# ofsoundof/NTIRE2022_ESR

Measured on AMD Instinct MI355X. Metric: images/sec (256x256->1024x1024 x4), higher is better.
Workload: dtype f32

## Files before the change

ntire2022_esr_amd/csrc/esr_wino.hip:

```cpp
#include <hip/hip_runtime.h>
#include <stddef.h>
#include <math.h>
#include <stdint.h>
#include <string.h>
#include <type_traits>

#include "esr_hip.h"
#include "esr_internal.h"

typedef float f32x4 __attribute__((ext_vector_type(4)));
typedef float f32x2 __attribute__((ext_vector_type(2)));
typedef int wn_i32x4 __attribute__((ext_vector_type(4)));

namespace {

constexpr int WN_THREADS = 256;
constexpr int WN_TILE = 16;
constexpr int WN_HALO = WN_TILE + 2;
constexpr int WN_PAIR = 37;
constexpr int WN_PLANE = 9 * WN_PAIR;
constexpr int WN_RAW_SLOTS = 2 * WN_PLANE;
constexpr int WN_LAST_LANES = WN_RAW_SLOTS - 640;
constexpr int WN_RAW_BYTES = WN_RAW_SLOTS * 16;
constexpr int WN_U_BYTES = 16 * 1024;
constexpr int WN_RING = 3;
constexpr int WN_RAW_OFF = WN_RING * WN_U_BYTES;
constexpr int WN_BIAS_OFF = WN_RAW_OFF + WN_RING * WN_RAW_BYTES;
constexpr int WN_LDS = WN_BIAS_OFF + 256;
static_assert(2 * WN_LDS <= 160 * 1024, "two blocks per CU");
constexpr int WN_MAX_BLOCKS = 512;
constexpr unsigned WN_OOB = 0x80000000u;
constexpr int WN_BARRIER_POS = 12;
constexpr int WN_FIRST_SHARE = 9;

struct WinoK {
    const float* x;
    const float* up;
    const float* bias;
    const float* res;
    float* y0;
    float* y1;
    int N, H, W;
    int nchunks, nhalves;
    unsigned up_bytes;
    int in_pitch, in_coff;
    int res_pitch, res_coff;
    int y0_pitch, y0_coff, y1_pitch, y1_coff;
    int cout_store, split;
    int act;
    float slope;
    int res_mode;
    int tiles_x, tiles_y;
    unsigned magic_x, magic_y;
    int y1_blk;
    int first_share;
    unsigned pix_floats;
    unsigned in_base;
    unsigned chunk_stride;
};

__device__ __forceinline__ unsigned wn_div(unsigned n, unsigned d, unsigned magic) { return d == 1 ? n : __umulhi(n, magic); }

__device__ __forceinline__ wn_i32x4 wn_rsrc(const void* base, size_t bytes)
{
    wn_i32x4 r;
    r.x = __builtin_amdgcn_readfirstlane((int)(size_t)base);
    r.y = __builtin_amdgcn_readfirstlane((int)(((size_t)base >> 32) & 0xffff));
    r.z = __builtin_amdgcn_readfirstlane((int)bytes);
    r.w = 0x00020000;
    return r;
}

template <int OFF>
__device__ __forceinline__ void wn_dma16(unsigned m0_base, unsigned voff, wn_i32x4 rsrc, unsigned soff)
{
    asm volatile("s_nop 0\n\tbuffer_load_dwordx4 %0, %1, %2 offen offset:%3 lds"
                 :: "v"(voff), "s"(rsrc), "s"(soff), "n"(OFF), "{m0}"(m0_base) : "memory");
}

__device__ __forceinline__ float wn_act1(float v, int act, float slope)
{
    switch (act) {
        case ESR_ACT_LRELU: return fmaxf(v, slope * v);
        case ESR_ACT_RELU: return fmaxf(v, 0.f);
        case ESR_ACT_GELU: return 0.5f * v * (1.f + erff(v * 0.70710678118654752440f));
        default: return v;
    }
}

template <int ACT>
__device__ __forceinline__ f32x4 wn_act4(f32x4 v, int act, float slope)
{
    if (ACT == ESR_ACT_LRELU) {
        const f32x4 m = v * slope;
        v.x = fmaxf(v.x, m.x); v.y = fmaxf(v.y, m.y); v.z = fmaxf(v.z, m.z); v.w = fmaxf(v.w, m.w);
    } else if (ACT < 0) {
        v.x = wn_act1(v.x, act, slope); v.y = wn_act1(v.y, act, slope);
        v.z = wn_act1(v.z, act, slope); v.w = wn_act1(v.w, act, slope);
    }
    return v;
}

__device__ __forceinline__ int wn_slot(int ly, int lx) { return (ly >> 1) * WN_PAIR + (ly & 1) * WN_HALO + lx; }

__device__ __forceinline__ f32x2 wn_lds_b64(unsigned addr)
{
    typedef const volatile __attribute__((address_space(3))) f32x2* lds_ptr;
    return *(lds_ptr)addr;
}

__device__ __forceinline__ f32x2 wn_sub2(f32x2 a, f32x2 b)
{
    f32x2 r;
    asm("v_pk_add_f32 %0, %1, %2 neg_lo:[0,1] neg_hi:[0,1]" : "=v"(r) : "v"(a), "v"(b));
    return r;
}

__device__ __forceinline__ void wn_pair_planes(f32x4& v0, f32x4& v1)
{
#pragma unroll
    for (int e = 0; e < 4; ++e) {
        const float a = v0[e], b = v1[e];
        const auto r = __builtin_amdgcn_permlane32_swap(__builtin_bit_cast(unsigned, a), __builtin_bit_cast(unsigned, b), false, false);
        const unsigned r0 = r[0], r1 = r[1];
        v0[e] = __builtin_bit_cast(float, r0);
        v1[e] = __builtin_bit_cast(float, r1);
    }
}

__device__ __forceinline__ f32x2 wn_add2(f32x2 a, f32x2 b)
{
    f32x2 r;
    asm("v_pk_add_f32 %0, %1, %2" : "=v"(r) : "v"(a), "v"(b));
    return r;
}

__device__ __forceinline__ void wn_mfma(f32x4& acc, float a, float b)
{
    asm("v_mfma_f32_16x16x4_f32 %0, %1, %2, %0" : "+v"(acc) : "v"(a), "v"(b));
}
__device__ __forceinline__ void wn_mfma_drain(f32x4& acc) { asm volatile("s_nop 15\n\ts_nop 3" : "+v"(acc)); }

#define WN_PIN(x) asm volatile("" : "+v"(x))

template <int ACT, int RES, int OUT>
__global__ __launch_bounds__(WN_THREADS, 2) void wino_f32_kernel(const WinoK p)
{
    __shared__ __attribute__((aligned(16))) char smem[WN_LDS];

    const int tid = threadIdx.x;
    const int lane = tid & 63;
    const int wv = __builtin_amdgcn_readfirstlane(tid >> 6);
    const int j = lane & 15, g = lane >> 4;
    const int tx = j & 7, ty = j >> 3;
    const unsigned smem_lds = (unsigned)(size_t)(__attribute__((address_space(3))) char*)smem;

    const int nwork = p.N * p.tiles_y * p.tiles_x * p.nhalves;
    const int G = gridDim.x;
    const bool classes = p.first_share != 8 && (G & 15) == 0;
    const int GC = classes ? G >> 1 : G;
    const bool second = classes && (int)blockIdx.x >= GC;
    const int n_first = classes ? (int)(((long)nwork * p.first_share / 16) & ~1L) : nwork;
    const int cbase = second ? n_first : 0, cend = second || !classes ? nwork : n_first;
    const int bl = second ? (int)blockIdx.x - GC : (int)blockIdx.x;
    auto work_index = [&](int k) -> int {
        const int base = cbase + k * GC;
        if (base >= cend) return -1;
        int off = bl;
        if ((GC & 7) == 0 && base + GC <= cend) off = (bl & 7) * (GC >> 3) + (bl >> 3);
        const int t = base + off;
        return t < cend ? t : -1;
    };

    struct Ctx { int n, x0, y0, half; unsigned voff[3]; };
    auto setup = [&](int work, Ctx& c) {
        if (work < 0) {
            c.n = 0; c.x0 = 0; c.y0 = 0; c.half = 0;
            c.voff[0] = c.voff[1] = c.voff[2] = WN_OOB;
            return;
        }
        const unsigned t = p.nhalves == 2 ? (unsigned)work >> 1 : (unsigned)work;
        c.half = p.nhalves == 2 ? work & 1 : 0;
        const unsigned tq = wn_div(t, (unsigned)p.tiles_x, p.magic_x);
        const unsigned txi = t - tq * p.tiles_x;
        c.n = (int)wn_div(tq, (unsigned)p.tiles_y, p.magic_y);
        const unsigned tyi = tq - (unsigned)c.n * p.tiles_y;
        c.x0 = (int)txi * WN_TILE;
        c.y0 = (int)tyi * WN_TILE;
#pragma unroll
        for (int i = 0; i < 3; ++i) {
            const int item = (wv * 3 + (wv == 3 && i == 2 ? 0 : i)) * 64 + lane;
            const int half = item >= WN_PLANE ? 1 : 0;
            const int slot = item - half * WN_PLANE;
            const int pr = slot / WN_PAIR, rem = slot - pr * WN_PAIR;
            const int odd = rem >= WN_HALO ? 1 : 0;
            const int ly = 2 * pr + odd, lx = rem - odd * WN_HALO;
            const int gy = c.y0 - 1 + ly, gx = c.x0 - 1 + lx;
            const bool ok = item < WN_RAW_SLOTS && rem < 2 * WN_HALO && gy >= 0 && gy < p.H && gx >= 0 && gx < p.W;
            c.voff[i] = (ok ? ((unsigned)(gy * p.W + gx) * p.pix_floats + 4u * half) * 4u + p.in_base : WN_OOB) - (i == 1 ? 1024u : 0u);
        }
    };
    const size_t img_bytes = (size_t)p.H * p.W * p.in_pitch * 4;
    const wn_i32x4 ursrc = wn_rsrc(p.up, p.up_bytes);
    const bool live1 = wv != 3 || lane < WN_LAST_LANES;
    const unsigned raw_m0 = smem_lds + (unsigned)(WN_RAW_OFF + wv * 3 * 1024);
    const unsigned raw_m0_2 = raw_m0 + (wv == 3 ? 0u : 2048u);
    const unsigned u_m0 = smem_lds + (unsigned)(wv * 4 * 1024);

    auto issue_raw = [&](int i, int rs, wn_i32x4 xr, int chunk, unsigned v) __attribute__((always_inline)) {
        const unsigned soff = (unsigned)chunk * p.chunk_stride;
        const unsigned ro = (unsigned)(rs * WN_RAW_BYTES);
        if (i == 0) wn_dma16<0>(raw_m0 + ro, v, xr, soff);
        else if (i == 1) { if (live1) wn_dma16<1024>(raw_m0 + ro, v, xr, soff); }
        else wn_dma16<0>(raw_m0_2 + ro, v, xr, soff);
    };
    auto image_rsrc = [&](int n) { return wn_rsrc(p.x + (size_t)n * (img_bytes / 4), img_bytes); };
    auto issue_u = [&](int i, int us, int half, int chunk, bool live) __attribute__((always_inline)) {
        const unsigned soff = (unsigned)((chunk * p.nhalves + half) * WN_U_BYTES + wv * 4 * 1024);
        const unsigned vo = live ? (unsigned)lane * 16u : WN_OOB;
        const unsigned m = u_m0 + (unsigned)(us * WN_U_BYTES);
        if (i == 0) wn_dma16<0>(m, vo, ursrc, soff);
        else if (i == 1) wn_dma16<1024>(m, vo, ursrc, soff);
        else if (i == 2) wn_dma16<2048>(m, vo, ursrc, soff);
        else wn_dma16<3072>(m, vo, ursrc, soff);
    };

    const int raw_lane = (g >> 1) * (WN_PLANE * 16) + wn_slot(4 * wv + 2 * ty, 2 * tx) * 16 + (g & 1) * 8;
    const int u_lane = lane * 16;

    auto raw_row = [&](unsigned rb, int r, f32x2 (&d)[4]) __attribute__((always_inline)) {
#pragma unroll
        for (int dx = 0; dx < 4; ++dx)
            d[dx] = wn_lds_b64(rb + ((r >> 1) * WN_PAIR + (r & 1) * WN_HALO + dx) * 16);
    };
    auto row_pass = [&](f32x2 (&V)[16], int r, const f32x2 (&d)[4]) __attribute__((always_inline)) {
        V[4 * r + 0] = wn_sub2(d[0], d[2]);
        V[4 * r + 1] = wn_add2(d[1], d[2]);
        V[4 * r + 2] = wn_sub2(d[2], d[1]);
        V[4 * r + 3] = wn_sub2(d[1], d[3]);
    };
    auto col_pass = [&](f32x2 (&V)[16], int c) __attribute__((always_inline)) {
        const f32x2 w0 = V[c], w1 = V[4 + c], w2 = V[8 + c], w3 = V[12 + c];
        V[c] = wn_sub2(w0, w2);
        V[4 + c] = wn_add2(w1, w2);
        V[8 + c] = wn_sub2(w2, w1);
        V[12 + c] = wn_sub2(w1, w3);
    };

    int k = 0;
    int work = work_index(0);
    if (work < 0) return;
    Ctx cur, nxt;
    setup(work, cur);
    int wn = work_index(1);
    setup(wn, nxt);

    {
        const wn_i32x4 xr = image_rsrc(cur.n);
#pragma unroll
        for (int c = 0; c < 3; ++c)
#pragma unroll
            for (int i = 0; i < 3; ++i) issue_raw(i, c, xr, c, cur.voff[i]);
#pragma unroll
        for (int i = 0; i < 4; ++i) issue_u(i, 0, cur.half, 0, true);
    }
    if (tid < p.nhalves * 8) *reinterpret_cast<f32x4*>(smem + WN_BIAS_OFF + tid * 16) = *reinterpret_cast<const f32x4*>(p.bias + tid * 4);
    asm volatile("s_waitcnt vmcnt(0) lgkmcnt(0)" ::: "memory");
    __builtin_amdgcn_s_barrier();
    f32x2 V0[16], V1[16];
    {
        unsigned rs = smem_lds + WN_RAW_OFF + raw_lane;
        asm volatile("" : "+v"(rs));
        f32x2 d[4];
#pragma unroll
        for (int r = 0; r < 4; ++r) { raw_row(rs, r, d); row_pass(V0, r, d); }
#pragma unroll
        for (int c = 0; c < 4; ++c) col_pass(V0, c);
    }
    asm volatile("s_waitcnt lgkmcnt(0)" ::: "memory");
    __builtin_amdgcn_s_barrier();
#pragma unroll
    for (int i = 0; i < 4; ++i) issue_u(i, 1, cur.half, 1, true);
    f32x4 a[4];
    a[0] = *reinterpret_cast<const f32x4*>(smem + u_lane);
    a[1] = *reinterpret_cast<const f32x4*>(smem + u_lane + 1024);

    int us = 0;
    int rsn = 1;

    f32x4 acc[16][2];
    for (;;) {
        const bool has_next = wn >= 0;
        f32x4 biasv[2];
#pragma unroll
        for (int ct = 0; ct < 2; ++ct) biasv[ct] = *reinterpret_cast<const f32x4*>(smem + WN_BIAS_OFF + (cur.half * 32 + ct * 16 + g * 4) * 4);

        auto stage = [&](auto first_tag, int c, f32x2 (&Vc)[16], f32x2 (&Vn)[16]) __attribute__((always_inline)) {
            constexpr bool FIRST = decltype(first_tag)::value;
            const bool rc = c + 3 < p.nchunks;
            const wn_i32x4 xr = image_rsrc(rc ? cur.n : nxt.n);
            const int rchunk = rc ? c + 3 : c + 3 - p.nchunks;
            int rs3 = rsn + 2;
            rs3 = rs3 >= 3 ? rs3 - 3 : rs3;
            const bool uc = c + 2 < p.nchunks;
            const int uhalf = uc ? cur.half : nxt.half, uchunk = uc ? c + 2 : c + 2 - p.nchunks;
            const bool ulive = uc || has_next;
            int us1 = us + 1, us2 = us + 2;
            us1 = us1 >= 3 ? us1 - 3 : us1;
            us2 = us2 >= 3 ? us2 - 3 : us2;
            const char* ust = smem + us * WN_U_BYTES + u_lane;
            const char* ust1 = smem + us1 * WN_U_BYTES + u_lane;
            unsigned rs = smem_lds + (unsigned)(WN_RAW_OFF + rsn * WN_RAW_BYTES) + raw_lane;
            asm volatile("" : "+v"(rs));
            f32x2 d[2][4];
#pragma unroll
            for (int pos = 0; pos < 16; ++pos) {
                if (pos == WN_BARRIER_POS) {
                    asm volatile("s_waitcnt vmcnt(3)" ::: "memory");
                    __builtin_amdgcn_s_barrier();
                }
                if (pos + 2 < 16) a[(pos + 2) & 3] = *reinterpret_cast<const f32x4*>(ust + (pos + 2) * 1024);
                else a[(pos + 2) & 3] = *reinterpret_cast<const f32x4*>(ust1 + (pos + 2 - 16) * 1024);
                if (pos < 4) raw_row(rs, pos, d[pos & 1]);
                if (pos >= 1 && pos < 5) {
                    row_pass(Vn, pos - 1, d[(pos - 1) & 1]);
#pragma unroll
                    for (int q = 0; q < 4; ++q) WN_PIN(Vn[4 * (pos - 1) + q]);
                }
                if (pos >= 5 && pos < 9) {
                    col_pass(Vn, pos - 5);
#pragma unroll
                    for (int q = 0; q < 4; ++q) WN_PIN(Vn[4 * q + pos - 5]);
                }
                if (pos == 2 || pos == 4 || pos == 6) {
                    const int i = pos / 2 - 1;
                    issue_raw(i, rs3, xr, rchunk, rc ? cur.voff[i] : nxt.voff[i]);
                }
                if (pos >= WN_BARRIER_POS) issue_u(pos - WN_BARRIER_POS, us2, uhalf, uchunk, ulive);
                const f32x4 zero = {0.f, 0.f, 0.f, 0.f};
                const f32x4 c0 = FIRST ? (pos == 5 ? biasv[0] : zero) : acc[pos][0];
                const f32x4 c1 = FIRST ? (pos == 5 ? biasv[1] : zero) : acc[pos][1];
                const f32x4 af = a[pos & 3];
                if (FIRST) {
                    acc[pos][0] = __builtin_amdgcn_mfma_f32_16x16x4f32(af.x, Vc[pos].x, c0, 0, 0, 0);
                    acc[pos][1] = __builtin_amdgcn_mfma_f32_16x16x4f32(af.z, Vc[pos].x, c1, 0, 0, 0);
                } else {
                    wn_mfma(acc[pos][0], af.x, Vc[pos].x);
                    wn_mfma(acc[pos][1], af.z, Vc[pos].x);
                }
                wn_mfma(acc[pos][0], af.y, Vc[pos].y);
                wn_mfma(acc[pos][1], af.w, Vc[pos].y);
                __builtin_amdgcn_sched_barrier(0);
            }
            us = us1;
            rsn = rsn == 2 ? 0 : rsn + 1;
        };
        stage(std::true_type{}, 0, V0, V1);
        stage(std::false_type{}, 1, V1, V0);
        for (int c = 2; c < p.nchunks; c += 2) {
            stage(std::false_type{}, c, V0, V1);
            stage(std::false_type{}, c + 1, V1, V0);
        }

        {
            wn_mfma_drain(acc[15][1]);
            const int ybase = cur.y0 + 4 * wv + 2 * ty, xbase = cur.x0 + 2 * tx;
            unsigned pix[2][2];
            bool pok[2][2];
#pragma unroll
            for (int a = 0; a < 2; ++a)
#pragma unroll
                for (int b = 0; b < 2; ++b) {
                    pok[a][b] = ybase + a < p.H && xbase + b < p.W;
                    pix[a][b] = (unsigned)((ybase + a) * p.W + xbase + b);
                }
            const size_t hw = (size_t)p.H * p.W;
#pragma unroll
            for (int ct = 0; ct < 2; ++ct) {
                const int cg = cur.half * 32 + ct * 16 + g * 4;
                const bool to0 = cur.half * 32 + ct * 16 < p.split;
                const bool cok = cg < p.cout_store;
                const int ch = to0 ? p.y0_coff + cg : p.y1_coff + cg - p.split;
                const bool blk = OUT == 1 && !to0;
                char* const dbase = reinterpret_cast<char*>(to0 ? p.y0 : p.y1) + (size_t)cur.n * hw * (size_t)((to0 ? p.y0_pitch : p.y1_pitch) * 4);
                const unsigned dps = blk ? 32u : (unsigned)((to0 ? p.y0_pitch : p.y1_pitch) * 4);
                const size_t dlane = blk ? (size_t)(ch >> 3) * hw * 32 + (size_t)(ch & 7) * 4 : (size_t)ch * 4;
                f32x4 rv[2][2];
                if (RES != ESR_RES_NONE) {
                    const char* rbase = reinterpret_cast<const char*>(p.res) + (size_t)cur.n * hw * (size_t)(p.res_pitch * 4) + (size_t)(p.res_coff + cg) * 4;
#pragma unroll
                    for (int a = 0; a < 2; ++a)
#pragma unroll
                        for (int b = 0; b < 2; ++b)
                            rv[a][b] = (pok[a][b] && cok) ? *reinterpret_cast<const f32x4*>(rbase + (size_t)pix[a][b] * (unsigned)(p.res_pitch * 4))
                                                          : f32x4{0.f, 0.f, 0.f, 0.f};
                }
                f32x4 Y[2][2];
#pragma unroll
                for (int jj = 0; jj < 4; ++jj) {
                    const f32x4 m0 = acc[jj][ct], m1 = acc[4 + jj][ct], m2 = acc[8 + jj][ct], m3 = acc[12 + jj][ct];
                    const f32x4 t0 = m0 + m1 + m2, t1 = m1 - m2 - m3;
                    if (jj == 0) { Y[0][0] = t0; Y[1][0] = t1; }
                    else if (jj == 1) { Y[0][0] += t0; Y[1][0] += t1; Y[0][1] = t0; Y[1][1] = t1; }
                    else if (jj == 2) { Y[0][0] += t0; Y[1][0] += t1; Y[0][1] -= t0; Y[1][1] -= t1; }
                    else { Y[0][1] -= t0; Y[1][1] -= t1; }
                }
                if (blk) {
                    char* const pa = dbase + (size_t)((p.y1_coff + cur.half * 32 + ct * 16 - p.split) >> 3) * hw * 32 + (size_t)(g & 1) * 16;
#pragma unroll
                    for (int a = 0; a < 2; ++a) {
                        f32x4 v0 = wn_act4<ACT>(Y[a][0], p.act, p.slope), v1 = wn_act4<ACT>(Y[a][1], p.act, p.slope);
                        wn_pair_planes(v0, v1);
                        const bool ok = (g >> 1) ? pok[a][1] : pok[a][0];
                        char* const q = pa + (size_t)((g >> 1) ? pix[a][1] : pix[a][0]) * 32;
                        if (ok) {
                            *reinterpret_cast<f32x4*>(q) = v0;
                            *reinterpret_cast<f32x4*>(q + hw * 32) = v1;
                        }
                    }
                } else
#pragma unroll
                for (int a = 0; a < 2; ++a)
#pragma unroll
                    for (int b = 0; b < 2; ++b) {
                        f32x4 v = Y[a][b];
                        if (RES == ESR_RES_PRE_ACT) v = wn_act4<ACT>(v + rv[a][b], p.act, p.slope);
                        else if (RES == ESR_RES_POST_ACT) v = wn_act4<ACT>(v, p.act, p.slope) + rv[a][b];
                        else v = wn_act4<ACT>(v, p.act, p.slope);
                        if (OUT == 2) {
                            const int cidx = cur.half * 2 + ct, nco = p.cout_store >> 4;
                            float* const o = p.y0 + ((size_t)(cur.n * nco + cidx) * (4 * p.H) + 4 * (ybase + a) + g) * (size_t)(4 * p.W) + 4 * (xbase + b);
                            if (pok[a][b] && cidx < nco) *reinterpret_cast<f32x4*>(o) = v;
                        } else if (pok[a][b] && cok) *reinterpret_cast<f32x4*>(dbase + dlane + (size_t)pix[a][b] * dps) = v;
                    }
            }
        }
        if (!has_next) break;
        cur = nxt;
        ++k;
        wn = work_index(k + 1);
        setup(wn, nxt);
    }
    asm volatile("s_waitcnt vmcnt(0)" ::: "memory");
}


constexpr int W8_THREADS = 512;
constexpr int W8_PLANE = 3 * WN_PAIR;
constexpr int W8_SLOTS = 2 * W8_PLANE;
constexpr int W8_SLOT_BYTES = W8_SLOTS * 16;
constexpr int W8_LAST_LANES = W8_SLOTS - 192;
constexpr int W8_EPI_STORES = 8;
constexpr int W8_MAX_BLOCKS = 256;
#ifndef W8_TP
#define W8_TP 2
#endif
#ifndef W8_DMA_TOP
#define W8_DMA_TOP 0
#endif
#ifndef W8_STAGGER
#define W8_STAGGER 0
#endif
#ifndef W8_ABL_NODMA
#define W8_ABL_NODMA 0
#endif
#ifndef W8_ABL_NOXF
#define W8_ABL_NOXF 0
#endif
#ifndef W8_ABL_NOA
#define W8_ABL_NOA 0
#endif
#ifndef W8_ABL_NOEPI
#define W8_ABL_NOEPI 0
#endif
#ifndef W8_ABL_NOMFMA
#define W8_ABL_NOMFMA 0
#endif
#ifndef W8_ABL_LAXWAIT
#define W8_ABL_LAXWAIT 0
#endif
#ifndef W8_ABL_OOBST
#define W8_ABL_OOBST 0
#endif
#ifndef W8_ABL_OOBDMA
#define W8_ABL_OOBDMA 0
#endif

template <int NCH> struct W8L {
    static constexpr int U_BYTES = NCH * WN_U_BYTES;
    static constexpr int RAW_OFF = U_BYTES;
    static constexpr int BIAS_OFF = RAW_OFF + 8 * 2 * W8_SLOT_BYTES;
    static constexpr int TOTAL = BIAS_OFF + 256;
    static_assert(TOTAL <= 160 * 1024, "one block per CU");
};

__device__ __forceinline__ void wn_store16(f32x4 v, unsigned voff, wn_i32x4 rsrc)
{
    asm volatile("buffer_store_dwordx4 %0, %1, %2, 0 offen\n\ts_nop 1" :: "v"(v), "v"(voff), "s"(rsrc) : "memory");
}

template <int ACT, int OUT, int NCH>
__global__ __launch_bounds__(W8_THREADS, 1) void wino8_f32_kernel(const WinoK p)
{
    typedef W8L<NCH> LY;
    __shared__ __attribute__((aligned(16))) char smem[LY::TOTAL];
    const int tid = threadIdx.x;
    const int lane = tid & 63;
    const int wv = __builtin_amdgcn_readfirstlane(tid >> 6);
    const int j = lane & 15, g = lane >> 4;
    const int tx = j & 7, ty = j >> 3;
    const unsigned smem_lds = (unsigned)(size_t)(__attribute__((address_space(3))) char*)smem;

    const int nh = p.nhalves;
    const int half = nh == 2 ? ((int)blockIdx.x >> 3) & 1 : 0;
    const int pidx = nh == 2 ? (((int)blockIdx.x >> 4) << 3) + ((int)blockIdx.x & 7) : (int)blockIdx.x;
    const int npair = nh == 2 ? (int)gridDim.x >> 1 : (int)gridDim.x;
    const int nstrips = p.N * p.tiles_y * p.tiles_x;
    const int per_block = (nstrips + npair - 1) / npair;
    const int s_end = min((pidx + 1) * per_block, nstrips);
    auto strip_index = [&](int k) -> int {
        const int s = pidx * per_block + k * 8 + wv;
        return s < s_end ? s : -1;
    };

    struct Ctx { int n, x0, y0; };
    unsigned dvoff[4];
    int dn = 0;
    auto locate = [&](int strip, Ctx& c) {
        if (strip < 0) { c.n = 0; c.x0 = 0; c.y0 = 0; return; }
        const unsigned sq = wn_div((unsigned)strip, (unsigned)p.tiles_x, p.magic_x);
        const unsigned sxi = (unsigned)strip - sq * p.tiles_x;
        c.n = (int)wn_div(sq, (unsigned)p.tiles_y, p.magic_y);
        const unsigned syi = sq - (unsigned)c.n * p.tiles_y;
        c.x0 = (int)sxi * 16;
        c.y0 = (int)syi * 4;
    };
    auto dma_to = [&](int strip, const Ctx& c) {
        dn = c.n;
        if (strip < 0) {
            dvoff[0] = dvoff[1] = dvoff[2] = dvoff[3] = WN_OOB;
            return;
        }
#pragma unroll
        for (int i = 0; i < 4; ++i) {
            const int item = i * 64 + lane;
            const int plane = item >= W8_PLANE ? 1 : 0;
            const int slot = item - plane * W8_PLANE;
            const int pr = slot / WN_PAIR, rem = slot - pr * WN_PAIR;
            const int odd = rem >= WN_HALO ? 1 : 0;
            const int ly = 2 * pr + odd, lx = rem - odd * WN_HALO;
            const int gy = c.y0 - 1 + ly, gx = c.x0 - 1 + lx;
            const bool ok = item < W8_SLOTS && rem < 2 * WN_HALO && gy >= 0 && gy < p.H && gx >= 0 && gx < p.W;
            dvoff[i] = ((ok && !W8_ABL_OOBDMA) ? ((unsigned)(gy * p.W + gx) * p.pix_floats + 4u * plane) * 4u + p.in_base : WN_OOB) - (unsigned)(i * 1024);
        }
    };
    const size_t img_bytes = (size_t)p.H * p.W * p.in_pitch * 4;
    auto image_rsrc = [&](int n) { return wn_rsrc(p.x + (size_t)n * (img_bytes / 4), img_bytes); };
    const unsigned ring_m0 = smem_lds + (unsigned)(LY::RAW_OFF + wv * 2 * W8_SLOT_BYTES);
    const bool live3 = lane < W8_LAST_LANES;
    auto issue_raw = [&](int par, int chunk) __attribute__((always_inline)) {
        const wn_i32x4 xr = image_rsrc(dn);
        const unsigned soff = (unsigned)chunk * p.chunk_stride;
        const unsigned m = ring_m0 + (unsigned)(par * W8_SLOT_BYTES);
        wn_dma16<0>(m, dvoff[0], xr, soff);
        wn_dma16<1024>(m, dvoff[1], xr, soff);
        wn_dma16<2048>(m, dvoff[2], xr, soff);
        if (live3) wn_dma16<3072>(m, dvoff[3], xr, soff);
    };

    int work = strip_index(0);
    {
        const wn_i32x4 ursrc = wn_rsrc(p.up, p.up_bytes);
#pragma unroll 1
        for (int pc = wv; pc < NCH * 16; pc += 8) {
            const int chunk = pc >> 4, piece = pc & 15;
            wn_dma16<0>(smem_lds + (unsigned)(chunk * WN_U_BYTES + piece * 1024), (unsigned)lane * 16u, ursrc,
                        (unsigned)((chunk * nh + half) * WN_U_BYTES + piece * 1024));
        }
        if (tid < nh * 8) *reinterpret_cast<f32x4*>(smem + LY::BIAS_OFF + tid * 16) = *reinterpret_cast<const f32x4*>(p.bias + tid * 4);
    }
    Ctx cur, nxt;
    locate(work, cur);
    int wn = strip_index(1);
    locate(wn, nxt);
    if (work >= 0) {
        dma_to(work, cur);
        issue_raw(0, 0);
        issue_raw(1, 1);
    }
    asm volatile("s_waitcnt vmcnt(0) lgkmcnt(0)" ::: "memory");
    __builtin_amdgcn_s_barrier();
    if (work < 0) return;

    const int raw_lane = (g >> 1) * (W8_PLANE * 16) + wn_slot(2 * ty, 2 * tx) * 16 + (g & 1) * 8;
    const int u_lane = lane * 16;
    auto raw_row = [&](unsigned rb, int r, f32x2 (&d)[4]) __attribute__((always_inline)) {
#pragma unroll
        for (int dx = 0; dx < 4; ++dx)
            d[dx] = wn_lds_b64(rb + ((r >> 1) * WN_PAIR + (r & 1) * WN_HALO + dx) * 16);
    };
    auto row_pass = [&](f32x2 (&V)[16], int r, const f32x2 (&d)[4]) __attribute__((always_inline)) {
        V[4 * r + 0] = wn_sub2(d[0], d[2]);
        V[4 * r + 1] = wn_add2(d[1], d[2]);
        V[4 * r + 2] = wn_sub2(d[2], d[1]);
        V[4 * r + 3] = wn_sub2(d[1], d[3]);
    };
    auto col_pass = [&](f32x2 (&V)[16], int c) __attribute__((always_inline)) {
        const f32x2 w0 = V[c], w1 = V[4 + c], w2 = V[8 + c], w3 = V[12 + c];
        V[c] = wn_sub2(w0, w2);
        V[4 + c] = wn_add2(w1, w2);
        V[8 + c] = wn_sub2(w2, w1);
        V[12 + c] = wn_sub2(w1, w3);
    };

    f32x2 V0[16], V1[16];
    {
        unsigned rs = ring_m0 + raw_lane;
        asm volatile("" : "+v"(rs));
        f32x2 d[4];
#pragma unroll
        for (int r = 0; r < 4; ++r) { raw_row(rs, r, d); row_pass(V0, r, d); }
#pragma unroll
        for (int c = 0; c < 4; ++c) col_pass(V0, c);
    }
    asm volatile("s_waitcnt lgkmcnt(0)" ::: "memory");
    if (!W8_DMA_TOP) issue_raw(0, 2);
    f32x4 a[4];
    a[0] = *reinterpret_cast<const f32x4*>(smem + u_lane);
    a[1] = *reinterpret_cast<const f32x4*>(smem + u_lane + 1024);

    if (W8_STAGGER > 0 && wv >= 4) {
#pragma unroll
        for (int i = 0; i < (W8_STAGGER + 126) / 127; ++i) __builtin_amdgcn_s_sleep(W8_STAGGER < 127 ? W8_STAGGER : 127);
    }
    int k = 0;
    f32x4 acc[16][2];
    if (W8_ABL_NOXF) {
#pragma unroll
        for (int q = 0; q < 16; ++q) V1[q] = V0[q];
    }
    if (W8_ABL_NOA) { a[2] = a[0]; a[3] = a[1]; }
    const char* const bias_lds = smem + LY::BIAS_OFF + (half * 32 + g * 4) * 4;
    for (;;) {
        const bool has_next = wn >= 0;
        auto stage = [&](auto first_tag, int c, f32x2 (&Vc)[16], f32x2 (&Vn)[16]) __attribute__((always_inline)) {
            constexpr bool FIRST = decltype(first_tag)::value;
            if (W8_DMA_TOP) {
                if (c + 2 == NCH) dma_to(wn, nxt);
                issue_raw(c & 1, c + 2 < NCH ? c + 2 : c + 2 - NCH);
            }
            f32x4 biasv0, biasv1;
            const int cn = c + 1 < NCH ? c + 1 : 0;
            const char* ust = smem + c * WN_U_BYTES + u_lane;
            const char* ust1 = smem + cn * WN_U_BYTES + u_lane;
            unsigned rs = ring_m0 + (unsigned)(((c + 1) & 1) * W8_SLOT_BYTES) + raw_lane;
            asm volatile("" : "+v"(rs));
            f32x2 d[2][4];
#pragma unroll
            for (int pos = 0; pos < 16; ++pos) {
                if (!W8_ABL_NOA) {
                if (pos + 2 < 16) a[(pos + 2) & 3] = *reinterpret_cast<const f32x4*>(ust + (pos + 2) * 1024);
                else a[(pos + 2) & 3] = *reinterpret_cast<const f32x4*>(ust1 + (pos + 2 - 16) * 1024);
                }
                if (pos == W8_TP) {
                    if (c < (W8_DMA_TOP ? 1 : 2) + 2 * W8_ABL_LAXWAIT && k > 0) asm volatile("s_waitcnt vmcnt(%0)" :: "n"(4 + W8_EPI_STORES) : "memory");
                    else asm volatile("s_waitcnt vmcnt(4)" ::: "memory");
                }
                if (!W8_DMA_TOP && pos == W8_TP + 5) {
                    if (c + 3 == NCH) dma_to(wn, nxt);
                    if (!W8_ABL_NODMA) issue_raw((c + 1) & 1, c + 3 < NCH ? c + 3 : c + 3 - NCH);
                }
                if (!W8_ABL_NOXF && pos >= W8_TP && pos < W8_TP + 4) raw_row(rs, pos - W8_TP, d[(pos - W8_TP) & 1]);
                if (!W8_ABL_NOXF && pos >= W8_TP + 1 && pos < W8_TP + 5) {
                    row_pass(Vn, pos - W8_TP - 1, d[(pos - W8_TP - 1) & 1]);
#pragma unroll
                    for (int q = 0; q < 4; ++q) WN_PIN(Vn[4 * (pos - W8_TP - 1) + q]);
                }
                if (!W8_ABL_NOXF && pos >= W8_TP + 5 && pos < W8_TP + 9) {
                    col_pass(Vn, pos - W8_TP - 5);
#pragma unroll
                    for (int q = 0; q < 4; ++q) WN_PIN(Vn[4 * q + pos - W8_TP - 5]);
                }
                if (FIRST && pos == 3) {
                    biasv0 = *reinterpret_cast<const f32x4*>(bias_lds);
                    biasv1 = *reinterpret_cast<const f32x4*>(bias_lds + 64);
                }
                const f32x4 zero = {0.f, 0.f, 0.f, 0.f};
                const f32x4 c0 = FIRST ? (pos == 5 ? biasv0 : zero) : acc[pos][0];
                const f32x4 c1 = FIRST ? (pos == 5 ? biasv1 : zero) : acc[pos][1];
                const f32x4 af = a[pos & 3];
                if (W8_ABL_NOMFMA) {
                    acc[pos][0] = c0; acc[pos][1] = c1;
                    acc[pos][0].x += af.x * Vc[pos].x + af.y * Vc[pos].y; acc[pos][1].x += af.z * Vc[pos].x + af.w * Vc[pos].y;
                } else if (FIRST) {
                acc[pos][0] = __builtin_amdgcn_mfma_f32_16x16x4f32(af.x, Vc[pos].x, c0, 0, 0, 0);
                acc[pos][1] = __builtin_amdgcn_mfma_f32_16x16x4f32(af.z, Vc[pos].x, c1, 0, 0, 0);
                wn_mfma(acc[pos][0], af.y, Vc[pos].y);
                wn_mfma(acc[pos][1], af.w, Vc[pos].y);
                } else {
                wn_mfma(acc[pos][0], af.x, Vc[pos].x);
                wn_mfma(acc[pos][1], af.z, Vc[pos].x);
                wn_mfma(acc[pos][0], af.y, Vc[pos].y);
                wn_mfma(acc[pos][1], af.w, Vc[pos].y);
                }
                __builtin_amdgcn_sched_barrier(0);
            }
        };
        stage(std::true_type{}, 0, V0, V1);
        stage(std::false_type{}, 1, V1, V0);
#pragma unroll
        for (int c = 2; c < NCH; c += 2) {
            stage(std::false_type{}, c, V0, V1);
            stage(std::false_type{}, c + 1, V1, V0);
        }

        if (W8_ABL_NOEPI) {
            if (p.N < 0) {
                f32x4 sum = {0.f, 0.f, 0.f, 0.f};
#pragma unroll
                for (int q = 0; q < 16; ++q) sum += acc[q][0] + acc[q][1];
                *reinterpret_cast<f32x4*>(p.y0 + lane * 4) = sum;
            }
        } else
        {
            wn_mfma_drain(acc[15][1]);
            const int ybase = cur.y0 + 2 * ty, xbase = cur.x0 + 2 * tx;
            const size_t hw = (size_t)p.H * p.W;
            unsigned pix[2][2];
            bool pok[2][2];
#pragma unroll
            for (int aa = 0; aa < 2; ++aa)
#pragma unroll
                for (int b = 0; b < 2; ++b) {
                    pok[aa][b] = ybase + aa < p.H && xbase + b < p.W;
                    pix[aa][b] = (unsigned)((ybase + aa) * p.W + xbase + b);
                }
#pragma unroll
            for (int ct = 0; ct < 2; ++ct) {
                const int cg = half * 32 + ct * 16 + g * 4;
                const bool to0 = half * 32 + ct * 16 < p.split;
                const bool cok = cg < p.cout_store;
                const int ch = to0 ? p.y0_coff + cg : p.y1_coff + cg - p.split;
                const bool blk = OUT == 1 && !to0;
                const unsigned pitch_b = (unsigned)((to0 ? p.y0_pitch : p.y1_pitch) * 4);
                const size_t ibytes = hw * pitch_b;
                const wn_i32x4 yr = wn_rsrc(reinterpret_cast<const char*>(to0 ? p.y0 : p.y1) + (size_t)cur.n * ibytes, ibytes);
                const unsigned dps = blk ? 32u : pitch_b;
                const unsigned dlane = blk ? (unsigned)(ch >> 3) * (unsigned)(hw * 32) + (unsigned)(ch & 7) * 4u : (unsigned)ch * 4u;
                f32x4 Y[2][2];
#pragma unroll
                for (int jj = 0; jj < 4; ++jj) {
                    const f32x4 m0 = acc[jj][ct], m1 = acc[4 + jj][ct], m2 = acc[8 + jj][ct], m3 = acc[12 + jj][ct];
                    const f32x4 t0 = m0 + m1 + m2, t1 = m1 - m2 - m3;
                    if (jj == 0) { Y[0][0] = t0; Y[1][0] = t1; }
                    else if (jj == 1) { Y[0][0] += t0; Y[1][0] += t1; Y[0][1] = t0; Y[1][1] = t1; }
                    else if (jj == 2) { Y[0][0] += t0; Y[1][0] += t1; Y[0][1] -= t0; Y[1][1] -= t1; }
                    else { Y[0][1] -= t0; Y[1][1] -= t1; }
                }
                if (blk) {
                    const unsigned plane_a = (unsigned)((p.y1_coff + half * 32 + ct * 16 - p.split) >> 3) * (unsigned)(hw * 32) + (unsigned)(g & 1) * 16u;
#pragma unroll
                    for (int aa = 0; aa < 2; ++aa) {
                        f32x4 v0 = wn_act4<ACT>(Y[aa][0], p.act, p.slope), v1 = wn_act4<ACT>(Y[aa][1], p.act, p.slope);
                        wn_pair_planes(v0, v1);
                        const bool ok = (g >> 1) ? pok[aa][1] : pok[aa][0];
                        const unsigned po = plane_a + ((g >> 1) ? pix[aa][1] : pix[aa][0]) * 32u;
                        wn_store16(v0, (ok && !W8_ABL_OOBST) ? po : WN_OOB, yr);
                        wn_store16(v1, (ok && !W8_ABL_OOBST) ? po + (unsigned)(hw * 32) : WN_OOB, yr);
                    }
                } else {
#pragma unroll
                for (int aa = 0; aa < 2; ++aa)
#pragma unroll
                    for (int b = 0; b < 2; ++b) {
                        const f32x4 v = wn_act4<ACT>(Y[aa][b], p.act, p.slope);
                        wn_store16(v, (pok[aa][b] && cok && !W8_ABL_OOBST) ? dlane + pix[aa][b] * dps : WN_OOB, yr);
                    }
                }
            }
        }
        if (!has_next) break;
        cur = nxt;
        ++k;
        wn = strip_index(k + 1);
        locate(wn, nxt);
    }
    asm volatile("s_waitcnt vmcnt(0)" ::: "memory");
}

template <int ACT, int OUT, int NCH>
int w8_launch(const WinoK& k, int grid, hipStream_t st)
{
    esr_note_kernel("wino8_f32_kernel<%d, %d, %d>", ACT, OUT, NCH);
    hipLaunchKernelGGL((wino8_f32_kernel<ACT, OUT, NCH>), dim3(grid), dim3(W8_THREADS), 0, st, k);
    esr_graph_note_io(st, k.x, offsetof(WinoK, x), k.y0, offsetof(WinoK, y0));
    return esr_check_launch("wino8_f32_kernel launch");
}

template <int ACT, int RES, int OUT>
int wn_launch(const WinoK& k, int grid, hipStream_t st)
{
    esr_note_kernel("wino_f32_kernel<%d, %d, %d>", ACT, RES, OUT);
    hipLaunchKernelGGL((wino_f32_kernel<ACT, RES, OUT>), dim3(grid), dim3(WN_THREADS), 0, st, k);
    esr_graph_note_io(st, k.x, offsetof(WinoK, x), k.y0, offsetof(WinoK, y0));
    return esr_check_launch("wino_f32_kernel launch");
}

bool g_wino8_enabled = true;

const double WN_G[4][3] = {{1.0, 0.0, 0.0}, {0.5, 0.5, 0.5}, {0.5, -0.5, 0.5}, {0.0, 0.0, 1.0}};

inline size_t wn_index(int nhalves, int slot, int pos, int o)
{
    const int chunk = slot / 8, within = slot % 8;
    const int kq = within / 2, s = within % 2;
    const int half = o / 32, ctl = (o % 32) / 16, i = o % 16;
    return ((((size_t)chunk * nhalves + half) * 16 + pos) * 64 + kq * 16 + i) * 4 + ctl * 2 + s;
}

}

int esr_wino_supported(const esr_conv_desc* d)
{
    if (!d || d->ksize != 3 || d->in_layout != ESR_NHWC) return 0;
    if (d->res_mode == ESR_RES_GATE) return 0;
    if (d->out_layout == ESR_NCHW_SHUFFLE4) {
        if ((d->cout & 15) || d->res_mode != ESR_RES_NONE || (d->split > 0 && d->split < d->cout) || (d->blocked8 & ESR_BLOCKED_OUT1)) return 0;
    } else if (d->out_layout != ESR_NHWC) return 0;
    if (d->storage != ESR_STORE_F32 || d->compute != ESR_COMPUTE_F32) return 0;
    if (d->tail_wpacked || d->post_wpacked || d->border_bias || d->in_seg_stride) return 0;
    if ((d->blocked8 & ESR_BLOCKED_OUT1) && d->res_mode != ESR_RES_NONE) return 0;
    if (d->cin <= 0 || d->cout <= 0 || d->cout > 64) return 0;
    const int cin_phys = esr_round_up(d->cin, 8);
    const int nchunks = cin_phys / 8;
    if (nchunks < 4 || (nchunks & 1)) return 0;
    if ((d->blocked8 & ESR_BLOCKED_IN) && !esr_view_aligned(d->in, 8)) return 0;
    if (d->blocked8 & ~(ESR_BLOCKED_IN | ESR_BLOCKED_OUT1)) return 0;
    if (d->hilo) return 0;
    const int cout4 = esr_round_up(d->cout, 4);
    int split = d->split <= 0 ? cout4 : d->split;
    if (split >= d->cout) split = cout4;
    if (split < cout4 && (split & 15)) return 0;
    const double tx = (d->w + 15) / 16, ty = (d->h + 15) / 16;
    if ((double)d->n * tx * ty * (tx > ty ? tx : ty) >= 4294967296.0) return 0;
    if ((double)d->h * d->w * d->in.pitch * 4.0 >= 2147482624.0) return 0;
    return 1;
}

extern "C" {

size_t esr_packed_wino_bytes(int cin_phys, int cout)
{
    if (cin_phys <= 0 || cout <= 0) return 0;
    const size_t nchunks = (size_t)esr_round_up(cin_phys, 8) / 8;
    const size_t nhalves = (size_t)esr_round_up(cout, 32) / 32;
    return (nchunks * nhalves * 16 * 256 + nhalves * 32) * sizeof(float);
}

int esr_pack_wino_f32(const float* w, const float* bias, int cin, int cout, const int32_t* cin_map, int cin_phys, void* out, size_t out_bytes)
{
    if (!w || !out || cin <= 0 || cout <= 0) return ESR_ERR_BAD_ARG;
    if (!cin_map && cin_phys < cin) return ESR_ERR_BAD_ARG;
    const size_t need = esr_packed_wino_bytes(cin_phys, cout);
    if (need == 0 || out_bytes < need) return ESR_ERR_BAD_ARG;
    const int nhalves = esr_round_up(cout, 32) / 32;
    float* o = static_cast<float*>(out);
    memset(o, 0, need);
    for (int s = 0; s < cin_phys; ++s) {
        const int c = cin_map ? cin_map[s] : (s < cin ? s : -1);
        if (c < 0) continue;
        if (c >= cin) return ESR_ERR_BAD_ARG;
        for (int oc = 0; oc < cout; ++oc) {
            const float* g = w + ((size_t)oc * cin + c) * 9;
            double t[4][3];
            for (int i = 0; i < 4; ++i)
                for (int b = 0; b < 3; ++b) t[i][b] = WN_G[i][0] * g[b] + WN_G[i][1] * g[3 + b] + WN_G[i][2] * g[6 + b];
            for (int i = 0; i < 4; ++i)
                for (int jj = 0; jj < 4; ++jj) {
                    const double u = t[i][0] * WN_G[jj][0] + t[i][1] * WN_G[jj][1] + t[i][2] * WN_G[jj][2];
                    o[wn_index(nhalves, s, 4 * i + jj, oc)] = (float)u;
                }
        }
    }
    float* bo = o + (size_t)(esr_round_up(cin_phys, 8) / 8) * nhalves * 16 * 256;
    if (bias)
        for (int oc = 0; oc < cout; ++oc) bo[oc] = bias[oc];
    return ESR_OK;
}

int esr_unpack_wino_f32(const void* packed, size_t bytes, int cin, int cout, const int32_t* cin_map, int cin_phys, float* u, float* bias)
{
    if (!packed || !u || cin <= 0 || cout <= 0) return ESR_ERR_BAD_ARG;
    if (bytes < esr_packed_wino_bytes(cin_phys, cout)) return ESR_ERR_BAD_ARG;
    const int nhalves = esr_round_up(cout, 32) / 32;
    const float* o = static_cast<const float*>(packed);
    memset(u, 0, sizeof(float) * (size_t)cout * cin * 16);
    for (int s = 0; s < cin_phys; ++s) {
        const int c = cin_map ? cin_map[s] : (s < cin ? s : -1);
        if (c < 0) continue;
        for (int oc = 0; oc < cout; ++oc)
            for (int pos = 0; pos < 16; ++pos) u[((size_t)oc * cin + c) * 16 + pos] = o[wn_index(nhalves, s, pos, oc)];
    }
    if (bias) {
        const float* bo = o + (size_t)(esr_round_up(cin_phys, 8) / 8) * nhalves * 16 * 256;
        for (int oc = 0; oc < cout; ++oc) bias[oc] = bo[oc];
    }
    return ESR_OK;
}

void esr_dbg_wino8(int on) { g_wino8_enabled = on != 0; }

}

int esr_conv2d_wino(const esr_conv_desc* d, void* hip_stream)
{
    const int cin_phys = esr_round_up(d->cin, 8);
    const int cout4 = esr_round_up(d->cout, 4);
    int split = d->split <= 0 ? cout4 : d->split;
    if (split >= d->cout) split = cout4;
    WinoK k;
    k.x = static_cast<const float*>(d->in.ptr);
    k.up = static_cast<const float*>(d->wino_wpacked);
    k.nchunks = cin_phys / 8;
    k.nhalves = esr_round_up(d->cout, 32) / 32;
    k.up_bytes = (unsigned)esr_packed_wino_bytes(cin_phys, d->cout);
    k.bias = k.up + (size_t)k.nchunks * k.nhalves * 16 * 256;
    k.res = static_cast<const float*>(d->res.ptr);
    k.y0 = static_cast<float*>(d->out0.ptr);
    k.y1 = static_cast<float*>(d->out1.ptr);
    k.N = d->n; k.H = d->h; k.W = d->w;
    k.in_pitch = d->in.pitch; k.in_coff = d->in.coff;
    k.res_pitch = d->res.pitch; k.res_coff = d->res.coff;
    k.y0_pitch = d->out0.pitch; k.y0_coff = d->out0.coff;
    k.y1_pitch = d->out1.pitch; k.y1_coff = d->out1.coff;
    k.cout_store = cout4;
    k.split = split;
    k.act = d->act; k.slope = d->slope; k.res_mode = d->res_mode;
    k.tiles_x = (d->w + WN_TILE - 1) / WN_TILE;
    k.tiles_y = (d->h + WN_TILE - 1) / WN_TILE;
    k.y1_blk = (d->blocked8 & ESR_BLOCKED_OUT1) ? 1 : 0;
    k.magic_x = k.tiles_x == 1 ? 0u : (unsigned)(0x100000000ull / (unsigned)k.tiles_x) + 1u;
    k.magic_y = k.tiles_y == 1 ? 0u : (unsigned)(0x100000000ull / (unsigned)k.tiles_y) + 1u;
    const long nwork = (long)k.N * k.tiles_x * k.tiles_y * k.nhalves;
    const int grid = nwork < WN_MAX_BLOCKS ? (int)nwork : WN_MAX_BLOCKS;
    k.first_share = (grid == WN_MAX_BLOCKS && nwork >= 8L * grid) ? WN_FIRST_SHARE : 8;
    hipStream_t st = static_cast<hipStream_t>(hip_stream);
    const int a = d->act;
    const bool blocked_in = (d->blocked8 & ESR_BLOCKED_IN) != 0;
    k.pix_floats = blocked_in ? 8u : (unsigned)d->in.pitch;
    k.in_base = blocked_in ? (unsigned)(d->in.coff / 8) * (unsigned)(d->h * d->w * 32) : (unsigned)d->in.coff * 4u;
    k.chunk_stride = blocked_in ? (unsigned)(d->h * d->w * 32) : 32u;
    if ((k.nchunks == 4 || k.nchunks == 6) && d->res_mode == ESR_RES_NONE && d->out_layout == ESR_NHWC && g_wino8_enabled) {
        const long sx = (d->w + 15) / 16, sy = (d->h + 3) / 4;
        const long nstrips = (long)k.N * sx * sy;
        const double out_bytes = (double)d->h * d->w * 4.0 * (d->out0.pitch > d->out1.pitch ? d->out0.pitch : d->out1.pitch);
        const bool fits = (double)k.N * sx * sy * (sx > sy ? sx : sy) < 4294967296.0 && out_bytes < 2147482624.0;
        if (fits && nstrips >= 4L * 8 * W8_MAX_BLOCKS / k.nhalves) {
            WinoK w = k;
            w.tiles_x = (int)sx; w.tiles_y = (int)sy;
            w.magic_x = sx == 1 ? 0u : (unsigned)(0x100000000ull / (unsigned)sx) + 1u;
            w.magic_y = sy == 1 ? 0u : (unsigned)(0x100000000ull / (unsigned)sy) + 1u;
            const int grid8 = W8_MAX_BLOCKS;
            const bool blk = k.y1_blk != 0;
            const bool lr = a == ESR_ACT_LRELU;
            if (k.nchunks == 6) {
                if (blk) return lr ? w8_launch<ESR_ACT_LRELU, 1, 6>(w, grid8, st) : w8_launch<-1, 1, 6>(w, grid8, st);
                return lr ? w8_launch<ESR_ACT_LRELU, 0, 6>(w, grid8, st) : w8_launch<-1, 0, 6>(w, grid8, st);
            }
            if (blk) return lr ? w8_launch<ESR_ACT_LRELU, 1, 4>(w, grid8, st) : w8_launch<-1, 1, 4>(w, grid8, st);
            return lr ? w8_launch<ESR_ACT_LRELU, 0, 4>(w, grid8, st) : w8_launch<-1, 0, 4>(w, grid8, st);
        }
    }
    if (d->out_layout == ESR_NCHW_SHUFFLE4)
        return a == ESR_ACT_NONE ? wn_launch<ESR_ACT_NONE, ESR_RES_NONE, 2>(k, grid, st) : wn_launch<-1, ESR_RES_NONE, 2>(k, grid, st);
    if (k.y1_blk)
        return a == ESR_ACT_LRELU ? wn_launch<ESR_ACT_LRELU, ESR_RES_NONE, 1>(k, grid, st) : wn_launch<-1, ESR_RES_NONE, 1>(k, grid, st);
    if (d->res_mode == ESR_RES_NONE)
        return a == ESR_ACT_LRELU ? wn_launch<ESR_ACT_LRELU, ESR_RES_NONE, 0>(k, grid, st)
             : a == ESR_ACT_NONE  ? wn_launch<ESR_ACT_NONE, ESR_RES_NONE, 0>(k, grid, st) : wn_launch<-1, ESR_RES_NONE, 0>(k, grid, st);
    if (d->res_mode == ESR_RES_PRE_ACT)
        return a == ESR_ACT_LRELU ? wn_launch<ESR_ACT_LRELU, ESR_RES_PRE_ACT, 0>(k, grid, st)
             : a == ESR_ACT_NONE  ? wn_launch<ESR_ACT_NONE, ESR_RES_PRE_ACT, 0>(k, grid, st) : wn_launch<-1, ESR_RES_PRE_ACT, 0>(k, grid, st);
    return a == ESR_ACT_LRELU ? wn_launch<ESR_ACT_LRELU, ESR_RES_POST_ACT, 0>(k, grid, st) : wn_launch<-1, ESR_RES_POST_ACT, 0>(k, grid, st);
}
```

Baseline: 1830.

## Skip MFMAs for padded output channel tiles and split w8 strips by wave groups

In the Winograd kernel, work items whose second 16-channel tile lies entirely beyond cout_store now skip the corresponding MFMAs and stores through a compile-time DEAD stage variant. The half index is XORed with the loop iteration so that dead halves alternate across consecutive work items. The w8 kernel gains a share-based split of strips between two groups of four waves, replacing round-robin assignment, using a default share of 11/16. Debug knobs for the w8 mode and its share are also added.

```diff
diff --git a/ntire2022_esr_amd/csrc/esr_wino.hip b/ntire2022_esr_amd/csrc/esr_wino.hip
--- a/ntire2022_esr_amd/csrc/esr_wino.hip
+++ b/ntire2022_esr_amd/csrc/esr_wino.hip
@@ -155,6 +155,7 @@
     const int tx = j & 7, ty = j >> 3;
     const unsigned smem_lds = (unsigned)(size_t)(__attribute__((address_space(3))) char*)smem;
 
+    constexpr bool SKIP = RES == ESR_RES_NONE && OUT != 1;
     const int nwork = p.N * p.tiles_y * p.tiles_x * p.nhalves;
     const int G = gridDim.x;
     const bool classes = p.first_share != 8 && (G & 15) == 0;
@@ -173,14 +174,14 @@
     };
 
     struct Ctx { int n, x0, y0, half; unsigned voff[3]; };
-    auto setup = [&](int work, Ctx& c) {
+    auto setup = [&](int work, int k, Ctx& c) {
         if (work < 0) {
             c.n = 0; c.x0 = 0; c.y0 = 0; c.half = 0;
             c.voff[0] = c.voff[1] = c.voff[2] = WN_OOB;
             return;
         }
         const unsigned t = p.nhalves == 2 ? (unsigned)work >> 1 : (unsigned)work;
-        c.half = p.nhalves == 2 ? work & 1 : 0;
+        c.half = p.nhalves == 2 ? (work ^ (SKIP ? k : 0)) & 1 : 0;
         const unsigned tq = wn_div(t, (unsigned)p.tiles_x, p.magic_x);
         const unsigned txi = t - tq * p.tiles_x;
         c.n = (int)wn_div(tq, (unsigned)p.tiles_y, p.magic_y);
@@ -251,9 +252,9 @@
     int work = work_index(0);
     if (work < 0) return;
     Ctx cur, nxt;
-    setup(work, cur);
+    setup(work, 0, cur);
     int wn = work_index(1);
-    setup(wn, nxt);
+    setup(wn, 1, nxt);
 
     {
         const wn_i32x4 xr = image_rsrc(cur.n);
@@ -291,12 +292,13 @@
     f32x4 acc[16][2];
     for (;;) {
         const bool has_next = wn >= 0;
+        const bool dead = SKIP && cur.half * 32 + 16 >= p.cout_store;
         f32x4 biasv[2];
 #pragma unroll
         for (int ct = 0; ct < 2; ++ct) biasv[ct] = *reinterpret_cast<const f32x4*>(smem + WN_BIAS_OFF + (cur.half * 32 + ct * 16 + g * 4) * 4);
 
-        auto stage = [&](auto first_tag, int c, f32x2 (&Vc)[16], f32x2 (&Vn)[16]) __attribute__((always_inline)) {
-            constexpr bool FIRST = decltype(first_tag)::value;
+        auto stage = [&](auto first_tag, auto dead_tag, int c, f32x2 (&Vc)[16], f32x2 (&Vn)[16]) __attribute__((always_inline)) {
+            constexpr bool FIRST = decltype(first_tag)::value, DEAD = decltype(dead_tag)::value;
             const bool rc = c + 3 < p.nchunks;
             const wn_i32x4 xr = image_rsrc(rc ? cur.n : nxt.n);
             const int rchunk = rc ? c + 3 : c + 3 - p.nchunks;
@@ -339,31 +341,41 @@
                 if (pos >= WN_BARRIER_POS) issue_u(pos - WN_BARRIER_POS, us2, uhalf, uchunk, ulive);
                 const f32x4 zero = {0.f, 0.f, 0.f, 0.f};
                 const f32x4 c0 = FIRST ? (pos == 5 ? biasv[0] : zero) : acc[pos][0];
-                const f32x4 c1 = FIRST ? (pos == 5 ? biasv[1] : zero) : acc[pos][1];
                 const f32x4 af = a[pos & 3];
                 if (FIRST) {
                     acc[pos][0] = __builtin_amdgcn_mfma_f32_16x16x4f32(af.x, Vc[pos].x, c0, 0, 0, 0);
-                    acc[pos][1] = __builtin_amdgcn_mfma_f32_16x16x4f32(af.z, Vc[pos].x, c1, 0, 0, 0);
+                    if (!DEAD) acc[pos][1] = __builtin_amdgcn_mfma_f32_16x16x4f32(af.z, Vc[pos].x, pos == 5 ? biasv[1] : zero, 0, 0, 0);
+                    else acc[pos][1] = zero;
                 } else {
                     wn_mfma(acc[pos][0], af.x, Vc[pos].x);
-                    wn_mfma(acc[pos][1], af.z, Vc[pos].x);
+                    if (!DEAD) wn_mfma(acc[pos][1], af.z, Vc[pos].x);
                 }
                 wn_mfma(acc[pos][0], af.y, Vc[pos].y);
-                wn_mfma(acc[pos][1], af.w, Vc[pos].y);
+                if (!DEAD) wn_mfma(acc[pos][1], af.w, Vc[pos].y);
                 __builtin_amdgcn_sched_barrier(0);
             }
             us = us1;
             rsn = rsn == 2 ? 0 : rsn + 1;
         };
-        stage(std::true_type{}, 0, V0, V1);
-        stage(std::false_type{}, 1, V1, V0);
-        for (int c = 2; c < p.nchunks; c += 2) {
-            stage(std::false_type{}, c, V0, V1);
-            stage(std::false_type{}, c + 1, V1, V0);
+        if (SKIP && dead) {
+            stage(std::true_type{}, std::true_type{}, 0, V0, V1);
+            stage(std::false_type{}, std::true_type{}, 1, V1, V0);
+            for (int c = 2; c < p.nchunks; c += 2) {
+                stage(std::false_type{}, std::true_type{}, c, V0, V1);
+                stage(std::false_type{}, std::true_type{}, c + 1, V1, V0);
+            }
+        } else {
+            stage(std::true_type{}, std::false_type{}, 0, V0, V1);
+            stage(std::false_type{}, std::false_type{}, 1, V1, V0);
+            for (int c = 2; c < p.nchunks; c += 2) {
+                stage(std::false_type{}, std::false_type{}, c, V0, V1);
+                stage(std::false_type{}, std::false_type{}, c + 1, V1, V0);
+            }
         }
 
         {
-            wn_mfma_drain(acc[15][1]);
+            if (SKIP && dead) wn_mfma_drain(acc[15][0]);
+            else wn_mfma_drain(acc[15][1]);
             const int ybase = cur.y0 + 4 * wv + 2 * ty, xbase = cur.x0 + 2 * tx;
             unsigned pix[2][2];
             bool pok[2][2];
@@ -377,6 +389,7 @@
             const size_t hw = (size_t)p.H * p.W;
 #pragma unroll
             for (int ct = 0; ct < 2; ++ct) {
+                if (SKIP && dead && ct == 1) break;
                 const int cg = cur.half * 32 + ct * 16 + g * 4;
                 const bool to0 = cur.half * 32 + ct * 16 < p.split;
                 const bool cok = cg < p.cout_store;
@@ -439,7 +452,7 @@
         cur = nxt;
         ++k;
         wn = work_index(k + 1);
-        setup(wn, nxt);
+        setup(wn, k + 1, nxt);
     }
     asm volatile("s_waitcnt vmcnt(0)" ::: "memory");
 }
@@ -452,6 +465,7 @@
 constexpr int W8_LAST_LANES = W8_SLOTS - 192;
 constexpr int W8_EPI_STORES = 8;
 constexpr int W8_MAX_BLOCKS = 256;
+constexpr int W8_OLD_SHARE = 11;
 #ifndef W8_TP
 #define W8_TP 2
 #endif
@@ -518,7 +532,14 @@
     const int nstrips = p.N * p.tiles_y * p.tiles_x;
     const int per_block = (nstrips + npair - 1) / npair;
     const int s_end = min((pidx + 1) * per_block, nstrips);
+    const int s_beg = min(pidx * per_block, s_end);
+    const int n_old = min(s_end - s_beg, ((int)((long)(s_end - s_beg) * p.first_share / 16) + 3) & ~3);
+    const int my_beg = wv < 4 ? s_beg : s_beg + n_old, my_end = wv < 4 ? s_beg + n_old : s_end;
     auto strip_index = [&](int k) -> int {
+        if (p.first_share != 8) {
+            const int s = my_beg + k * 4 + (wv & 3);
+            return s < my_end ? s : -1;
+        }
         const int s = pidx * per_block + k * 8 + wv;
         return s < s_end ? s : -1;
     };
@@ -806,7 +827,8 @@
     return esr_check_launch("wino_f32_kernel launch");
 }
 
-bool g_wino8_enabled = true;
+int g_wino8_mode = 1;
+int g_wino8_share = 0;
 
 const double WN_G[4][3] = {{1.0, 0.0, 0.0}, {0.5, 0.5, 0.5}, {0.5, -0.5, 0.5}, {0.0, 0.0, 1.0}};
 
@@ -908,7 +930,8 @@
     return ESR_OK;
 }
 
-void esr_dbg_wino8(int on) { g_wino8_enabled = on != 0; }
+void esr_dbg_wino8(int on) { g_wino8_mode = on < 0 || on > 2 ? 1 : on; }
+void esr_dbg_wino8_share(int s) { g_wino8_share = s >= 1 && s <= 15 ? s : 0; }
 
 }
 
@@ -950,16 +973,17 @@
     k.pix_floats = blocked_in ? 8u : (unsigned)d->in.pitch;
     k.in_base = blocked_in ? (unsigned)(d->in.coff / 8) * (unsigned)(d->h * d->w * 32) : (unsigned)d->in.coff * 4u;
     k.chunk_stride = blocked_in ? (unsigned)(d->h * d->w * 32) : 32u;
-    if ((k.nchunks == 4 || k.nchunks == 6) && d->res_mode == ESR_RES_NONE && d->out_layout == ESR_NHWC && g_wino8_enabled) {
+    if ((k.nchunks == 4 || k.nchunks == 6) && d->res_mode == ESR_RES_NONE && d->out_layout == ESR_NHWC && g_wino8_mode) {
         const long sx = (d->w + 15) / 16, sy = (d->h + 3) / 4;
         const long nstrips = (long)k.N * sx * sy;
         const double out_bytes = (double)d->h * d->w * 4.0 * (d->out0.pitch > d->out1.pitch ? d->out0.pitch : d->out1.pitch);
         const bool fits = (double)k.N * sx * sy * (sx > sy ? sx : sy) < 4294967296.0 && out_bytes < 2147482624.0;
-        if (fits && nstrips >= 4L * 8 * W8_MAX_BLOCKS / k.nhalves) {
+        if (fits && (nstrips >= 4L * 8 * W8_MAX_BLOCKS / k.nhalves || g_wino8_mode == 2)) {
             WinoK w = k;
             w.tiles_x = (int)sx; w.tiles_y = (int)sy;
             w.magic_x = sx == 1 ? 0u : (unsigned)(0x100000000ull / (unsigned)sx) + 1u;
             w.magic_y = sy == 1 ? 0u : (unsigned)(0x100000000ull / (unsigned)sy) + 1u;
+            w.first_share = g_wino8_share ? g_wino8_share : W8_OLD_SHARE;
             const int grid8 = W8_MAX_BLOCKS;
             const bool blk = k.y1_blk != 0;
             const bool lr = a == ESR_ACT_LRELU;
```

New measurement: 1852 (median of 6 runs). 1.01x the previous value.
